# jiahuei/COMIC-Compact-Image-Captioning-with-Attention

Hardware: AMD Instinct MI355X
Metric: images/sec (decoder-mode XE training, COMIC-256, InceptionV3 frozen) (higher is better)
Workload: dtype bf16

## Files before the change

### comic-compact-image-captioning-with-attention_amd/_lib.py

```python
import ctypes as C
import os

_HERE = os.path.dirname(os.path.abspath(__file__))
LIB_PATH = os.environ.get('COMIC_HIP_LIB') or os.path.join(_HERE, 'lib', 'libcomic_hip.so')

c_void_p, c_int, c_int32, c_int64, c_float, c_double, c_char_p, c_uint64 = (
    C.c_void_p, C.c_int, C.c_int32, C.c_int64, C.c_float, C.c_double, C.c_char_p, C.c_uint64)


class CnnOp(C.Structure):
    _fields_ = [(n, c_int32) for n in (
        'kind', 'src', 'dst', 'src_coff', 'dst_coff', 'H', 'W', 'Cin', 'Cout', 'KH', 'KW', 'SH', 'SW',
        'PT', 'PL', 'Ho', 'Wo', 'weight', 'relu', 'out_f32', 'src_f32', 'lane', 'tile', 'group', 'flags', 'min_lds')]


class ImageDesc(C.Structure):
    _fields_ = [('offset', C.c_int64), ('in_h', c_int32), ('in_w', c_int32), ('flip', c_int32), ('oy', c_int32),
                ('ox', c_int32), ('sy', C.c_float), ('sx', C.c_float)]


class ImageAug(C.Structure):
    _fields_ = [('mode', c_int32), ('cy', c_int32), ('cx', c_int32), ('ch', c_int32), ('cw', c_int32), ('sy', C.c_float),
                ('sx', C.c_float), ('ops', C.c_uint8 * 4), ('brightness', C.c_float), ('saturation', C.c_float),
                ('hue', C.c_float), ('contrast', C.c_float)]
# ... 40 lines not shown
            ('COMIC_BWD_OWN_ROWS', '1', DEC_BWD_OWN_ROWS))


def decoder_flags_from_env():
    f = 0
    for name, val, bit in _DEC_ENV:
        if os.environ.get(name, '')[:1] == val:
            f |= bit
    return f


CONV_TILES = 61
WS_TILE = 54
IMG_TILE = 55
CHAIN_TILE = 62
OP_RAW, OP_POOLED_SRC, OP_X3 = 1, 2, 4
OP_CHAIN_LINK = 8
OP_CHAIN_KEEP = 16
IM2COL_CONV_TILES = 12


def is_im2col_tile(tile):
    return tile <= IM2COL_CONV_TILES or 26 <= tile <= 47
PARAM_NAMES = ('W_init', 'K', 'b', 'W_m', 'W_v', 'W_q', 'v', 'ln_g', 'ln_b', 'tau', 'W_a', 'W_o', 'b_o', 'emb', 'cell_ln', 'K_c', 'b_c', 'status')


class DecoderParams(C.Structure):
    _fields_ = [(n, c_void_p) for n in PARAM_NAMES]


# ... 329 lines not shown
```

### comic-compact-image-captioning-with-attention_amd/csrc/conv.hip

```cpp
#include "conv_run.h"
#include "conv_ws.h"
#include "conv_stem.h"
#include "conv_img.h"
#include <cstdlib>
#include <cstring>
#include <algorithm>
#include <vector>

namespace {

template <typename T, int BM, int BN, int WM, int WN, bool MASK = false>
__global__ __launch_bounds__(256) void conv_igemm_kernel(ConvArgs a) {
  constexpr int EPC = Elem<T>::EPC;
  constexpr int BKE = 4 * EPC;
  constexpr int A_PASSES = (BM + 63) / 64;
  constexpr int B_PASSES = (BN + 63) / 64;
  constexpr int TM = BM / WM / 16;
  constexpr int TN = BN / WN / 16;
  static_assert(WM * WN == 4, "4 waves");

  __shared__ __attribute__((aligned(16))) unsigned char smem[2 * (BM + BN) * kRowBytes];
  unsigned char* Xs = smem;
  unsigned char* Ws = smem + 2 * BM * kRowBytes;

// ... 1564 lines not shown
    if (img_config(a[j]) != cfg || !img_same_shape(a[j], a[0])) {
      comic_set_error("conv: the members of an image-resident launch must have one shape");
      return 3;
    }
    ComicImgMember& m = ia.m[j];
    m.x = (const bf16_t*)a[j].x; m.wf = (const bf16_t*)a[j].w_frag; m.scale = a[j].scale; m.shift = a[j].shift; m.y = a[j].y;
    m.x_cs = a[j].x_cs; m.x_co = a[j].x_co; m.y_cs = a[j].y_cs; m.y_co = a[j].y_co;
    m.KH = a[j].KH; m.KW = a[j].KW; m.PT = a[j].PT; m.PL = a[j].PL; m.relu = a[j].relu; m.out_f32 = a[j].out_f32;
  }
  return comic_img_launch(cfg, ia, st);
}

int validate_grouped_conv(const comic_cnn_op* op, int xc, int yc, const comic_conv_weight* wt, int batch);
template <typename HT>
int launch_img_chains(const comic_cnn_op* op, int n, void* const* buffers, const int32_t* buf_channels,
                      const comic_conv_weight* weights, int batch, hipStream_t st) {
  ComicChainArgs ca;
  memset(&ca, 0, sizeof(ca));
  ca.f16 = std::is_same<HT, f16_t>::value;
  ca.B = batch; ca.H = op[0].H; ca.W = op[0].W; ca.Cin = op[0].Cin;
  const int pxb = ca.Cin * 2;
  ca.PXBp = pxb + ((pxb % 64 == 0) ? 32 : 0);
  COMIC_REQUIRE(comic_img_chain_supported(ca.H, ca.W, ca.Cin), "conv chain: %dx%d maps of %d channels are not supported", ca.H,
                ca.W, ca.Cin);
  int nm = 0;
  for (int j = 0; j < n;) {
    COMIC_REQUIRE(nm < kChainMaxMembers, "conv chain: more than %d chains in one launch", kChainMaxMembers);
    ComicChainMember& m = ca.m[nm];
    int len = 0;
    for (;; ++len) {
      COMIC_REQUIRE(j + len < n && len < kChainMaxConvs, "conv chain: a chain of more than %d convs, or a link flag on the last op",
                    kChainMaxConvs);
      const comic_cnn_op* o = op + j + len;
      const comic_conv_weight* wt = weights + o->weight;
      const bool link = (o->flags & COMIC_OP_CHAIN_LINK) != 0;
      if (int rc = validate_grouped_conv(o, buf_channels[o->src], buf_channels[o->dst], wt, batch)) return rc;
      COMIC_REQUIRE(o->SH == 1 && o->SW == 1 && o->Ho == o->H && o->Wo == o->W && o->H == ca.H && o->W == ca.W &&
                        o->Cin == ca.Cin && o->KH * o->KW >= 2 && o->KH * o->KW <= 32 && !(o->flags & (COMIC_OP_RAW | COMIC_OP_X3)),
                    "conv chain: every conv must be a stride-1 SAME conv with BatchNorm over the chain's %dx%dx%d input", ca.H, ca.W,
                    ca.Cin);
// ... 11 lines not shown
        COMIC_REQUIRE(buffers[o->dst] && buf_channels[o->dst] % 4 == 0, "conv chain: a kept intermediate map needs its buffer");
        c.keep = buffers[o->dst]; c.keep_cs = buf_channels[o->dst]; c.keep_co = o->dst_coff;
      }
      if (len == 0) {
        COMIC_REQUIRE(buf_channels[o->src] % 8 == 0 && o->src_coff % 8 == 0 && buffers[o->src], "conv chain: bad source slice");
        m.x = (const bf16_t*)buffers[o->src]; m.x_cs = buf_channels[o->src]; m.x_co = o->src_coff;
      }
      if (!link) {
        COMIC_REQUIRE(buffers[o->dst], "conv chain: null destination");
        m.y = buffers[o->dst]; m.y_cs = buf_channels[o->dst]; m.y_co = o->dst_coff; m.out_f32 = o->out_f32;
        ++len;
        break;
      }
    }
    m.n_convs = len;
    j += len;
    ++nm;
  }
  if (nm == 2 && ca.m[1].n_convs > ca.m[0].n_convs) std::swap(ca.m[0], ca.m[1]);
  ca.n_members = nm;
  return comic_img_chain_launch(ca, st);
}

constexpr int kNumConvTiles = 12;
constexpr int kWideTile0 = 26, kNumWideTiles = 22;
constexpr int kWalkTile0 = 56, kNumWalkTiles = 6;
inline int walk_split(int t) { return t >= kWalkTile0 + 3 ? 2 : 1; }
inline bool is_walk_tile(int t) { return t >= kWalkTile0 && t < kWalkTile0 + kNumWalkTiles; }
inline bool is_im2col_tile(int t) { return t <= kNumConvTiles || (t >= kWideTile0 && t < kWideTile0 + kNumWideTiles) || is_walk_tile(t); }
template <typename HT>
int launch_dma_tile(int tile, const ConvArgs& a, hipStream_t st) {
  switch (tile) {
    case 26: return launch_dma<HT, 128, 128, 2, 2, 2>(a, st);
// ... 174 lines not shown
    t0 += q.Cout / 16;
  }
  a.n_tiles = t0;
  if (int rc = comic_ws_launch(a, st)) return rc;
  COMIC_LAUNCH_CHECK("conv_ws");
  return 0;
}
bool ws_group_selected(const comic_cnn_op* ops, int n, int batch) {
  if (!ws_group_eligible(ops, n)) return false;
  if (ops[0].flags & COMIC_OP_POOLED_SRC) return true;
  if (ops[0].tile == COMIC_WS_TILE) return true;
  return ops[0].tile == 0 && (long)batch * ops[0].Ho * ops[0].Wo >= 64L * 256;
}

int group_tile(const comic_cnn_op* ops, int n, int batch) {
  if (ops[0].tile == COMIC_IMG_TILE || ops[0].tile == COMIC_CHAIN_TILE) return ops[0].tile;
  if (ops[0].tile > 0 && ops[0].tile < COMIC_WS_TILE) return ops[0].tile;
  if (is_walk_tile(ops[0].tile)) return ops[0].tile;
  bool all128 = true;
  for (int i = 0; i < n; ++i) all128 = all128 && ops[i].Cout % 128 == 0;
  auto blocks = [&](int t) {
    long b = 0;
    for (int i = 0; i < n; ++i)
      b += (long)cdiv(batch * ops[i].Ho * ops[i].Wo, kTileBM[t]) * cdiv(ops[i].Cout, kTileBN[t]);
    return b;
  };
  if (all128 && blocks(1) >= 512) return 1;
  if (blocks(2) >= 512) return 2;
  if (blocks(3) >= 384) return 3;
  return 4;
}
// ... 317 lines not shown
    if (ops[i].group <= 0) {
      ++i;
      continue;
    }
    if (ws_group_selected(ops + i, n, batch)) {
      memset(out, 0, sizeof(ConvArgs) * n);
      out += n;
      i += n;
      continue;
    }
    COMIC_REQUIRE(ops[i].tile != COMIC_WS_TILE, "conv: group is not eligible for the weight-stationary 1x1 kernel");
    const int tile = group_tile(ops + i, n, batch);
    for (int j = 0; j < n; ++j)
      COMIC_REQUIRE(tile == COMIC_CHAIN_TILE || !(ops[i + j].flags & COMIC_OP_CHAIN_LINK),
                    "conv: COMIC_OP_CHAIN_LINK ops depend on each other -- their group runs on COMIC_CHAIN_TILE only (got tile %d)", tile);
    if (tile == COMIC_IMG_TILE || tile == COMIC_CHAIN_TILE) {
      memset(out, 0, sizeof(ConvArgs) * n);
      out += n;
      i += n;
      continue;
    }
    int blk = 0;
    for (int j = 0; j < n; ++j) {
      const comic_cnn_op* op = ops + i + j;
      const comic_conv_weight* wt = weights + op->weight;
      if (int rc = validate_grouped_conv(op, buf_channels[op->src], buf_channels[op->dst], wt, batch)) return rc;
      COMIC_REQUIRE(buffers[op->src] && buffers[op->dst], "grouped conv: null buffer");
      ConvArgs& a = out[j];
      fill_args(a, op, buffers[op->src], buf_channels[op->src], buffers[op->dst], buf_channels[op->dst], wt, batch);
      COMIC_REQUIRE(a.zero, "conv: zero page symbol not resolvable");
      a.member_kind = op->kind == 7 ? 1 : 0;
// ... 107 lines not shown
    if (gargs && op->group > 0) {
      COMIC_REQUIRE(dtype == Half16<HT>::code && (op->kind == 0 || op->kind == 7) && op->lane == 0,
                    "grouped launch needs a bf16 or f16 plan and conv / pool+bn ops on the caller's stream");
      const int n = group_run(ops, n_ops, i);
      if (ws_group_selected(op, n, batch)) {
        if (int rc = run_ws_group<HT>(op, n, buffers, buf_channels, weights, batch, main_st)) return rc;
        gargs += n;
        i += n - 1;
        continue;
      }
      COMIC_REQUIRE(op->tile != COMIC_WS_TILE, "conv: group is not eligible for the weight-stationary 1x1 kernel");
      const int tile = group_tile(op, n, batch);
      for (int j = 0; j < n; ++j)
        COMIC_REQUIRE(tile == COMIC_CHAIN_TILE || !(op[j].flags & COMIC_OP_CHAIN_LINK),
                      "conv: COMIC_OP_CHAIN_LINK ops depend on each other -- their group runs on COMIC_CHAIN_TILE only (got tile %d)", tile);
      if (tile == COMIC_CHAIN_TILE) {
        if (int rc = launch_img_chains<HT>(op, n, buffers, buf_channels, weights, batch, main_st)) return rc;
        COMIC_LAUNCH_CHECK("image-resident conv chains");
        gargs += n;
        i += n - 1;
        continue;
      }
      if (tile == COMIC_IMG_TILE) {
        COMIC_REQUIRE(n <= kImgMaxMembers, "grouped launch: too many members for the image-resident kernel");
        ConvArgs ma[kImgMaxMembers];
        bool done[kImgMaxMembers] = {false, false, false, false};
        for (int j = 0; j < n; ++j) {
          COMIC_REQUIRE(op[j].kind == 0, "grouped launch: the image-resident kernel takes convolutions only");
          if (int rc = validate_grouped_conv(op + j, buf_channels[op[j].src], buf_channels[op[j].dst], weights + op[j].weight, batch)) return rc;
          fill_args(ma[j], op + j, buffers[op[j].src], buf_channels[op[j].src], buffers[op[j].dst], buf_channels[op[j].dst],
// ... 186 lines not shown
```

### comic-compact-image-captioning-with-attention_amd/csrc/conv_img.h

```cpp
#pragma once
#include "conv_common.h"

constexpr int kImgMaxMembers = 4;

struct ComicImgMember {
  const bf16_t* x;
  const bf16_t* wf;
  const float* scale;
  const float* shift;
  void* y;
  int x_cs, x_co, y_cs, y_co;
  int KH, KW, PT, PL, relu, out_f32;
};
struct ComicImgArgs {
  ComicImgMember m[kImgMaxMembers];
  int n_members;
  int B, H, W, Cin, Cout;
  int G, groups;
  int PXBp;
  int KS32;
  int f16;
};

int comic_img_config(int H, int W, int Cin, int Cout, int KH, int KW, int SH, int SW, int Ho, int Wo);
// ... 2 lines not shown

constexpr int kChainMaxConvs = 4, kChainMaxMembers = 2;
struct ComicChainConv {
  const bf16_t* wf;
  const float* scale;
  const float* shift;
  int KH, KW, PT, PL, KS32, Cout, relu, keep_cs;
  void* keep;
  int keep_co, pad_;
};
struct ComicChainMember {
  const bf16_t* x;
  void* y;
  int x_cs, x_co, y_cs, y_co, out_f32, n_convs;
  ComicChainConv c[kChainMaxConvs];
};
struct ComicChainArgs {
  ComicChainMember m[kChainMaxMembers];
  int n_members;
  int B, H, W, Cin, PXBp;
  int f16;
};
int comic_img_chain_supported(int H, int W, int Cin);
int comic_img_chain_launch(const ComicChainArgs& a, hipStream_t st);
```

### comic-compact-image-captioning-with-attention_amd/csrc/conv_img.hip

```cpp
#include <algorithm>

#include "conv_img.h"

namespace {

typedef __attribute__((ext_vector_type(4))) unsigned img_u32x4;

__device__ __forceinline__ __amdgpu_buffer_rsrc_t img_rsrc(const void* p, uint32_t bytes) {
  return __builtin_amdgcn_make_buffer_rsrc((void*)p, 0, (int)bytes, 0x00020000);
}

constexpr int img_zero_bytes(int cs) { return (256 + cs * 64 + 1023) / 1024 * 1024; }

template <int TM>
__device__ __forceinline__ void img_pixel_state(int lane, int wm, int P, int H, int W, int PXBp, int KH, int KW, int PT, int PL,
                                                int img0, uint32_t (&pixaddr)[TM], uint32_t (&mask)[TM], int (&mrow)[TM]) {
  const int fr = lane & 15, fg = lane >> 4;
  const int HW = H * W;
  const float rHW = 1.0f / (float)HW, rW = 1.0f / (float)W;
#pragma unroll
  for (int j = 0; j < TM; ++j) {
    const int p = (wm * TM + j) * 16 + fr;
    const bool pv = p < P;
    const int pp = pv ? p : 0;
// ... 118 lines not shown

  const int fg = lane >> 4;
  uint32_t pixaddr[TM], mask[TM];
  int mrow[TM];
  img_pixel_state<TM>(lane, wm, P, a.H, a.W, PXBp, m.KH, m.KW, m.PT, m.PL, img0, pixaddr, mask, mrow);
  f32x4_t acc[TN][TM];
  img_kloop<HT, TM, TN, CS, PD, true>(smem, zoff, pixaddr, mask, m.wf, a.Cout, a.KS32, m.KH, m.KW, m.PT, m.PL, a.W, PXBp, wn, lane, acc);

  ConvArgs ca;
  ca.scale = m.scale; ca.shift = m.shift; ca.y = m.y; ca.y_cs = m.y_cs; ca.y_co = m.y_co; ca.Cout = a.Cout;
  ca.relu = m.relu; ca.out_f32 = m.out_f32; ca.accum = 0; ca.x3 = 0; ca.x3_src = 0;
  ca.mask_y = nullptr;
  conv_store_tiles<HT, TN, TM>(ca, acc, wn * TN * 16, fg * 4, mrow);
}

template <typename HT, int TM, int TNI, int CS, int PD = 2>
__global__ __launch_bounds__(256, 2) void conv_img_chain_kernel(const ComicChainArgs a) {
  constexpr int NT = 256, WN = 4;
  constexpr int CPP = CS * 4;
  constexpr int PMAX = TM * 16;
  extern __shared__ __attribute__((aligned(16))) unsigned char smem[];
  const int tid = threadIdx.x, lane = tid & 63;
  const int wn = __builtin_amdgcn_readfirstlane(tid >> 6);
  const int mi = (int)blockIdx.x >= a.B ? 1 : 0;
  const int img0 = (int)blockIdx.x - mi * a.B;
  const ComicChainMember& m = a.m[mi];
  const int HW = a.H * a.W;
  const int P = HW;
  const int PXBp = a.PXBp;
  const uint32_t zoff = (PMAX * PXBp + 255) & ~255;

  {
    constexpr int U = (PMAX * CPP + NT - 1) / NT;
    const bf16_t* __restrict__ xg = m.x + (size_t)img0 * HW * m.x_cs + m.x_co;
    const int x_cs = m.x_cs;
    const int total = P * CPP;
    uint4 v[U];
    int dst[U];
#pragma unroll
    for (int u = 0; u < U; ++u) {
      const int idx = u * NT + tid;
      const bool ok = idx < total;
      const int p = ok ? idx / CPP : 0;
      const int c = ok ? idx - p * CPP : 0;
      dst[u] = ok ? p * PXBp + c * 16 : -1;
      v[u] = *(const uint4*)(xg + (size_t)p * x_cs + c * 8);
    }
#pragma unroll
    for (int u = 0; u < U; ++u)
      if (dst[u] >= 0) *(uint4*)(smem + dst[u]) = v[u];
    for (int z = tid; z < img_zero_bytes(CS) / 16; z += NT) *(uint4*)(smem + zoff + z * 16) = make_uint4(0u, 0u, 0u, 0u);
  }
  __syncthreads();

  const int fr = lane & 15, fg = lane >> 4;
  uint32_t pixaddr[TM], mask[TM];
  int mrow[TM];
  const int nc = m.n_convs;
  for (int ci = 0; ci + 1 < nc; ++ci) {
    const ComicChainConv& c = m.c[ci];
    img_pixel_state<TM>(lane, 0, P, a.H, a.W, PXBp, c.KH, c.KW, c.PT, c.PL, img0, pixaddr, mask, mrow);
    f32x4_t acc[TNI][TM];
    img_kloop<HT, TM, TNI, CS, PD, false>(smem, zoff, pixaddr, mask, c.wf, a.Cin, c.KS32, c.KH, c.KW, c.PT, c.PL, a.W, PXBp, wn, lane, acc);
    float4 sc[TNI], sh[TNI];
    bool nv[TNI];
#pragma unroll
    for (int i = 0; i < TNI; ++i) {
      nv[i] = (wn * TNI + i) * 16 < a.Cin;
      const int n0 = nv[i] ? (wn * TNI + i) * 16 + fg * 4 : 0;
      sc[i] = *(const float4*)(c.scale + n0);
      sh[i] = *(const float4*)(c.shift + n0);
    }
    const float lo = c.relu ? 0.f : -INFINITY;
    __syncthreads();
#pragma unroll
    for (int j = 0; j < TM; ++j) {
      unsigned char* prow = smem + (j * 16 + fr) * PXBp + (wn * TNI * 16 + fg * 4) * 2;
#pragma unroll
      for (int i = 0; i < TNI; ++i) {
        float v0 = fmaf(acc[i][j][0], sc[i].x, sh[i].x);
        float v1 = fmaf(acc[i][j][1], sc[i].y, sh[i].y);
        float v2 = fmaf(acc[i][j][2], sc[i].z, sh[i].z);
        float v3 = fmaf(acc[i][j][3], sc[i].w, sh[i].w);
        asm("v_max_f32 %0, %1, %2" : "=v"(v0) : "v"(v0), "s"(lo));
        asm("v_max_f32 %0, %1, %2" : "=v"(v1) : "v"(v1), "s"(lo));
        asm("v_max_f32 %0, %1, %2" : "=v"(v2) : "v"(v2), "s"(lo));
        asm("v_max_f32 %0, %1, %2" : "=v"(v3) : "v"(v3), "s"(lo));
        const uint2 pk = make_uint2(Half16<HT>::pack(v0, v1), Half16<HT>::pack(v2, v3));
        if (nv[i]) *(uint2*)(prow + i * 32) = pk;
        if (c.keep && nv[i])
          *(uint2*)((unsigned char*)c.keep + ((size_t)(img0 * HW + j * 16 + fr) * c.keep_cs + c.keep_co + (wn * TNI + i) * 16 + fg * 4) * 2) = pk;
      }
    }
    __syncthreads();
  }
  {
    const ComicChainConv& c = m.c[nc - 1];
    img_pixel_state<TM>(lane, 0, P, a.H, a.W, PXBp, c.KH, c.KW, c.PT, c.PL, img0, pixaddr, mask, mrow);
    f32x4_t acc[3][TM];
    img_kloop<HT, TM, 3, CS, PD, false>(smem, zoff, pixaddr, mask, c.wf, c.Cout, c.KS32, c.KH, c.KW, c.PT, c.PL, a.W, PXBp, wn, lane, acc);
    ConvArgs ca;
    ca.scale = c.scale; ca.shift = c.shift; ca.y = m.y; ca.y_cs = m.y_cs; ca.y_co = m.y_co; ca.Cout = c.Cout;
    ca.relu = c.relu; ca.out_f32 = m.out_f32; ca.accum = 0; ca.x3 = 0; ca.x3_src = 0;
    ca.mask_y = nullptr;
    conv_store_tiles<HT, 3, TM>(ca, acc, wn * 3 * 16, fg * 4, mrow);
  }
}

__global__ void pack_frag_kernel(const bf16_t* __restrict__ src, bf16_t* __restrict__ dst, const long* __restrict__ table,
// ... 39 lines not shown
  if (!attr_set) {
    if (hipFuncSetAttribute((const void*)conv_img_kernel<HT, TM, TN, WM, WN, CS, PD>, hipFuncAttributeMaxDynamicSharedMemorySize,
                            160 * 1024) != hipSuccess) {
      comic_set_error("conv_img: cannot reserve %d bytes of LDS", lds);
      return 1;
    }
    attr_set = true;
  }
  hipLaunchKernelGGL((conv_img_kernel<HT, TM, TN, WM, WN, CS, PD>), dim3(a.groups * a.n_members), dim3(64 * WM * WN), lds, st, a);
  return 0;
}

template <typename HT, int TNI, int CS>
int launch_chain(const ComicChainArgs& a, hipStream_t st) {
  constexpr int TM = 9;
  const int lds = ((TM * 16 * a.PXBp + 255) & ~255) + img_zero_bytes(CS);
  static PerDeviceOnce attr_once__;
  bool& attr_set = attr_once__.slot();
  if (!attr_set) {
    if (hipFuncSetAttribute((const void*)conv_img_chain_kernel<HT, TM, TNI, CS>, hipFuncAttributeMaxDynamicSharedMemorySize,
                            160 * 1024) != hipSuccess) {
      comic_set_error("conv_img_chain: cannot reserve %d bytes of LDS", lds);
      return 1;
    }
    attr_set = true;
  }
  hipLaunchKernelGGL((conv_img_chain_kernel<HT, TM, TNI, CS>), dim3(a.B * a.n_members), dim3(256), lds, st, a);
  return 0;
}

}
// ... 71 lines not shown
```

### comic-compact-image-captioning-with-attention_amd/nets.py

```python
from __future__ import annotations

import ctypes as C
import json
import math
import os

import numpy as np

from . import _lib as L
from . import streams

BN_EPS = 1e-3

_STEM = [('c', 'Conv2d_1a_3x3', 32, (3, 3), 2, 'VALID'), ('c', 'Conv2d_2a_3x3', 32, (3, 3), 1, 'VALID'),
         ('c', 'Conv2d_2b_3x3', 64, (3, 3), 1, 'SAME'), ('max', 'MaxPool_3a_3x3'),
         ('c', 'Conv2d_3b_1x1', 80, (1, 1), 1, 'VALID'), ('c', 'Conv2d_4a_3x3', 192, (3, 3), 1, 'VALID'),
         ('max', 'MaxPool_5a_3x3')]


def _c(scope, cout, k, stride=1, pad='SAME'):
    return ('c', scope, cout, k if isinstance(k, tuple) else (k, k), stride, pad)


def _mixed5(pool_c, b1):
# ... 67 lines not shown
            and 2 * (32 + 64) * 4 + 2 * 4 * 132 * 96 + 16 * Wi * 3 * 4 <= 160 * 1024)


def _out(size, k, s, pad):
    if pad == 'SAME':
        o = -(-size // s)
        tot = max((o - 1) * s + k - size, 0)
        return o, tot // 2
    return (size - k) // s + 1, 0


class CnnPlan:

    def __init__(self, name='inception_v3', image_size=(224, 224), final_endpoint='Mixed_7c', branch_streams=False,
                 group_branches=True, layers=None, pool_after_projection=False, ride_pools=False, side_pools=None,
                 fuse_pools=False, x3=False, fuse_stem_1a=True, fuse_chains=None):
        if name not in ('inception_v3', 'inception_v1', 'chain'):
            raise NotImplementedError('only inception_v3 / inception_v1 are on the MI355X hot path (got %r)' % name)
        self.name = name
        self.ops = []
        self.buffers = []
        self.weights = []
        self.wphys = []
        self.fm_src = None
        self.end_points = {}
        self.macs = 0
        self._lane = 0
        self._branch = None
        self.branch_streams = branch_streams
        self.group_branches = group_branches and not branch_streams
        self._depth = 0
        self._next_group = 1
        self.pool_after_projection = pool_after_projection
        self.ride_pools = ride_pools
        self.side_pools = bool(side_pools)
        self.fuse_pools = bool(fuse_pools)
        self.fuse_stem_1a = bool(fuse_stem_1a)
        bf16_grouped = not x3 and self.group_branches and name == 'inception_v3' and not self.ride_pools
        self.fuse_chains = bf16_grouped if fuse_chains is None else bool(fuse_chains)
        self.keep_chain_maps = not self.pool_after_projection
        self.small_batch_plan = None
        if fuse_chains is None and self.fuse_chains:
            self.small_batch_plan = CnnPlan(name, image_size, final_endpoint, branch_streams, group_branches, layers,
                                            pool_after_projection, ride_pools, side_pools, fuse_pools, x3, fuse_stem_1a,
                                            fuse_chains=False)
        if self.fuse_chains and (x3 or not self.group_branches):
            raise ValueError('fuse_chains needs a grouped bf16 plan')
        if self.fuse_pools and not (pool_after_projection and name == 'inception_v3'):
            raise ValueError('fuse_pools needs an inception_v3 plan with pool_after_projection=True')
        self._pooled_src = None
        self._logical = {}
        self.block_ranges = []
        if name == 'chain':
            self._build_chain(image_size, layers)
        elif name == 'inception_v1':
# ... 91 lines not shown
                             KH=k, KW=k, SH=stride, SW=stride, PT=pt, PL=pl, Ho=Ho, Wo=Wo, weight=-1, relu=0,
                             out_f32=0, lane=self._lane, depth=self._depth, branch=self._branch))
        return dst, (Ho, Wo, Cc)

    def _schedule_by_depth(self, first_op):
        block = self.ops[first_op:]
        del self.ops[first_op:]
        forked = False
        chains = self._find_chains(block) if self.fuse_chains else []
        chained = [o for ch in chains for o in ch]
        for ch in chains:
            rest = sorted((o for o in block if o.get('branch') == ch[0].get('branch') and o['depth'] > ch[-1]['depth']),
                          key=lambda o: o['depth'])
            for k, o in enumerate(rest):
                o['depth'] = ch[0]['depth'] + k
        block = [o for o in block if not any(o is c for c in chained)]
        for di, d in enumerate(sorted({o['depth'] for o in block})):
            if di == 1 and chains:
                self._emit_chains(chains)
                chains = []
            level = [o for o in block if o['depth'] == d]
            riders = [o for o in level if o['kind'] == 7] if self.ride_pools else []
            for o in level:
                if o['kind'] != 0 and o not in riders:
                    if o['kind'] == 7 and self.side_pools:
                        o['lane'] = 1
                        self.ops.append(self._sync_op(5))
                        forked = True
                    self.ops.append(o)
            convs = sorted((o for o in level if o['kind'] == 0), key=lambda o: -(o['KH'] * o['KW'] * o['Cin']))
            if not convs:
                self.ops += riders
                continue
            members = convs + riders
            if len(members) >= 2:
                for o in members:
                    o['group'] = self._next_group
                self._next_group += 1
            self.ops += members
        if chains:
            self._emit_chains(chains)
        if forked:
            self.ops.append(self._sync_op(6))

    CHAIN_CHANNELS = (128, 160, 192)
    CHAIN_MIN_BATCH = 96

    def _find_chains(self, block):
        def seven(o, cin):
            return (o['kind'] == 0 and o['H'] * o['W'] == 144 and (o['Ho'], o['Wo']) == (o['H'], o['W']) and
                    o['SH'] == o['SW'] == 1 and o['KH'] * o['KW'] == 7 and o['Cin'] == cin and not o.get('flags', 0))
        out = []
        for b in sorted({o.get('branch') for o in block if o.get('branch') is not None}):
            ops = sorted((o for o in block if o.get('branch') == b), key=lambda o: o['depth'])
            if len(ops) < 3 or ops[0]['kind'] != 0:
                continue
# ... 2 lines not shown
            for o in ops[1:]:
                if not (cin in self.CHAIN_CHANNELS and seven(o, cin) and len(run) < 4):
                    break
                if run and not (run[-1]['Cout'] == cin and not run[-1]['out_f32'] and run[-1]['dst'] == o['src']
                                and run[-1]['dst_coff'] == 0 and sum(1 for q in block if q['src'] == run[-1]['dst']) == 1):
                    break
                run.append(o)
            while run and run[-1]['Cout'] != 192:
                run.pop()
            if len(run) >= 2:
                out.append(run)
        if len(out) > 2 or len({ch[0]['Cin'] for ch in out}) > 1:
            return []
        return out

    def _emit_chains(self, chains):
        for ch in chains:
            for o in ch[:-1]:
                o['flags'] = o.get('flags', 0) | L.OP_CHAIN_LINK | (L.OP_CHAIN_KEEP if self.keep_chain_maps else 0)
            for o in ch:
                o['group'] = self._next_group
                o['tile'] = L.CHAIN_TILE
                self.ops.append(o)
        self._next_group += 1

    @staticmethod
    def _sync_op(kind):
        z = dict.fromkeys(('src', 'dst', 'src_coff', 'dst_coff', 'H', 'W', 'Cin', 'Cout', 'KH', 'KW', 'SH', 'SW', 'PT',
                           'PL', 'Ho', 'Wo', 'relu', 'out_f32'), 0)
        z.update(kind=kind, weight=-1, lane=0)
        return z
# ... 377 lines not shown
        self._train = None
        torch.cuda.synchronize()
        self._wt = wt
        self.bufs = []
        for (H, W, Cc, f32) in plan.buffers:
            self.bufs.append(torch.empty((batch, H, W, Cc), dtype=torch.float32 if f32 else tdt, device=device))
        self._bufptr = (C.c_void_p * len(self.bufs))(*[b.data_ptr() for b in self.bufs])
        self._bufch = (C.c_int32 * len(self.bufs))(*[b[2] for b in plan.buffers])
        ops = (L.CnnOp * len(plan.ops))()
        for i, o in enumerate(plan.ops):
            for k, v in o.items():
                if k not in ('depth', 'branch', 'block_in'):
                    setattr(ops[i], k, v)
            if not self.half:
                ops[i].group = 0
                if o.get('tile') == L.CHAIN_TILE:
                    ops[i].tile = 0
                    ops[i].flags &= ~(L.OP_CHAIN_LINK | L.OP_CHAIN_KEEP)
        self._ops = ops
        self._group_args = None
        self._build_group_args()
        self._graph = None
        self._calls = 0
        self._alt = {}
        self._last_bufptr = None
        self.backward_lanes = True
        self.backward_branch_lanes = True
        self._polite_lds_kb = 0
        self._fm_f32 = None

    @property
# ... 401 lines not shown
            src = self.bufs[self.plan.fm_src]
            if self._fm_f32 is None:
                self._fm_f32 = self.torch.empty(src.shape, dtype=self.torch.float32, device=self.device)
            self._fm_f32.copy_(src)
            fm = self._fm_f32
        else:
            fm = self.bufs[self.plan.fm]
        return pooled.reshape(B, -1), fm.reshape(B, fm.shape[1] * fm.shape[2], fm.shape[3])

    def _tune_key(self):
        p = self.plan
        H, W = p.buffers[p.input][:2]
        return '%s:%dx%d:B%d:%s%s:%dops:polite%d' % (p.name, H, W, self.batch, 'par' if p.pool_after_projection else 'plain',
                                                    ('+fp' if getattr(p, 'fuse_pools', False) else '') +
                                                    ('+ch' if getattr(p, 'fuse_chains', False) else '') +
                                                    ('+x3' if getattr(p, 'x3', False) else ''),
                                                  len(p.ops), self.polite_lds_kb) + (':f16' if self.dtype == 'f16' else '')

    def autotune(self, reps=5, verbose=False, cache=None):
        if not self.half:
            return {}
        torch = self.torch
        st = L.stream_ptr()
        if cache and os.path.isfile(cache):
            tiles = json.load(open(cache)).get(self._tune_key())
            if tiles is not None and len(tiles) == len(self.plan.ops):
                for i, t in enumerate(tiles):
                    self._ops[i].tile = int(t)
                if self._group_args is not None:
                    self._build_group_args()
# ... 9 lines not shown
        ev0, ev1 = torch.cuda.Event(enable_timing=True), torch.cuda.Event(enable_timing=True)
        n_ops = len(self.plan.ops)
        grouped = self._group_args is not None
        rec_bytes = 0
        if grouped:
            n_rec = sum(1 for j in range(n_ops) if self._ops[j].group > 0)
            rec_bytes = self.lib.comic_cnn_group_args_bytes(self._ops, n_ops) // n_rec
        rec = 0
        i = 0
        while i < n_ops:
            o = self.plan.ops[i]
            if o['kind'] != 0:
                i += 1
                continue
            op = self._ops[i]
            if o.get('flags', 0) & L.OP_POOLED_SRC or o.get('tile') == L.CHAIN_TILE:
                n = 1
                while i + n < n_ops and op.group > 0 and self._ops[i + n].group == op.group:
                    n += 1
                rec += n if (grouped and op.group > 0) else 0
                i += n
                continue
            n = 1
            if grouped and op.group > 0:
                while i + n < n_ops and self._ops[i + n].group == op.group:
                    n += 1
                first = C.byref(self._ops, i * C.sizeof(L.CnnOp))
                rec_off = rec * rec_bytes

                def run():
                    L.check(self.lib.comic_cnn_forward_grouped(first, n, self._bufptr, self._bufch, self._wt,
# ... 83 lines not shown
```

### include/comic_hip.h

```cpp
#ifndef COMIC_HIP_H_
#define COMIC_HIP_H_

#include <stddef.h>
#include <stdint.h>

#ifdef __cplusplus
extern "C" {
#endif

#define COMIC_F32 0
#define COMIC_BF16 1
#define COMIC_F16 2
#define COMIC_ABI_VERSION 1
#define COMIC_CONV_TILES 61
#define COMIC_WS_TILE 54
#define COMIC_IMG_TILE 55
#define COMIC_CHAIN_TILE 62

const char* comic_last_error(void);
int comic_abi_version(void);
int comic_device_count(void);


int comic_pack_conv_weights(const float* w_hwio, void* w_packed, int kh, int kw, int cin, int cout,
                            int dtype, void* stream);

int comic_fold_bn(const float* beta, const float* mean, const float* var, float eps, float* scale,
                  float* shift, int c, void* stream);

typedef struct comic_cnn_op {
  int32_t kind;
  int32_t src, dst;
// ... 597 lines not shown
```

Baseline: 40330.

## Fuse 1x1 head convs into image-resident conv chain kernels

```diff
diff --git a/comic-compact-image-captioning-with-attention_amd/_lib.py b/comic-compact-image-captioning-with-attention_amd/_lib.py
--- a/comic-compact-image-captioning-with-attention_amd/_lib.py
+++ b/comic-compact-image-captioning-with-attention_amd/_lib.py
@@ -78,6 +78,7 @@
 WS_TILE = 54
 IMG_TILE = 55
 CHAIN_TILE = 62
+CHAIN_HEAD_TILE = 63
 OP_RAW, OP_POOLED_SRC, OP_X3 = 1, 2, 4
 OP_CHAIN_LINK = 8
 OP_CHAIN_KEEP = 16
diff --git a/comic-compact-image-captioning-with-attention_amd/csrc/conv.hip b/comic-compact-image-captioning-with-attention_amd/csrc/conv.hip
--- a/comic-compact-image-captioning-with-attention_amd/csrc/conv.hip
+++ b/comic-compact-image-captioning-with-attention_amd/csrc/conv.hip
@@ -1602,7 +1602,8 @@
 int validate_grouped_conv(const comic_cnn_op* op, int xc, int yc, const comic_conv_weight* wt, int batch);
 template <typename HT>
 int launch_img_chains(const comic_cnn_op* op, int n, void* const* buffers, const int32_t* buf_channels,
-                      const comic_conv_weight* weights, int batch, hipStream_t st) {
+                      const comic_conv_weight* weights, int batch, hipStream_t st, const comic_cnn_op* heads = nullptr,
+                      int n_heads = 0) {
   ComicChainArgs ca;
   memset(&ca, 0, sizeof(ca));
   ca.f16 = std::is_same<HT, f16_t>::value;
@@ -1611,7 +1612,7 @@
   ca.PXBp = pxb + ((pxb % 64 == 0) ? 32 : 0);
   COMIC_REQUIRE(comic_img_chain_supported(ca.H, ca.W, ca.Cin), "conv chain: %dx%d maps of %d channels are not supported", ca.H,
                 ca.W, ca.Cin);
-  int nm = 0;
+  int nm = 0, heads_used = 0;
   for (int j = 0; j < n;) {
     COMIC_REQUIRE(nm < kChainMaxMembers, "conv chain: more than %d chains in one launch", kChainMaxMembers);
     ComicChainMember& m = ca.m[nm];
@@ -1653,9 +1654,40 @@
       }
     }
     m.n_convs = len;
+    for (int h = 0; h < n_heads; ++h) {
+      const comic_cnn_op* o = heads + h;
+      if (o->dst != op[j].src) continue;
+      const comic_conv_weight* wt = weights + o->weight;
+      COMIC_REQUIRE(!m.head.wf, "conv chain: two heads write the input of one chain");
+      if (int rc = validate_grouped_conv(o, buf_channels[o->src], buf_channels[o->dst], wt, batch)) return rc;
+      COMIC_REQUIRE(o->kind == 0 && o->KH == 1 && o->KW == 1 && o->SH == 1 && o->SW == 1 && o->PT == 0 && o->PL == 0 &&
+                        o->H == ca.H && o->W == ca.W && o->Ho == ca.H && o->Wo == ca.W && o->Cout == ca.Cin &&
+                        o->Cin % kChainHeadKT == 0 && !(o->flags & ~COMIC_OP_CHAIN_KEEP) && !o->out_f32 && o->dst_coff == 0 &&
+                        buf_channels[o->dst] == ca.Cin,
+                    "conv chain: a head must be a stride-1 1x1 conv with BatchNorm from a multiple of %d channels to the chain's %dx%dx%d map",
+                    kChainHeadKT, ca.H, ca.W, ca.Cin);
+      COMIC_REQUIRE(wt->w_frag, "conv chain: no fragment-order weights");
+      COMIC_REQUIRE(buffers[o->src] && buf_channels[o->src] % 8 == 0 && o->src_coff % 8 == 0 &&
+                        o->src_coff + o->Cin <= buf_channels[o->src],
+                    "conv chain: bad source slice of a head");
+      ComicChainConv& c = m.head;
+      c.wf = (const bf16_t*)wt->w_frag; c.scale = wt->scale; c.shift = wt->shift;
+      c.KH = 1; c.KW = 1; c.PT = 0; c.PL = 0; c.Cout = o->Cout; c.relu = o->relu;
+      c.KS32 = ((o->Cin + 63) / 64 * 64) / 32;
+      c.keep = nullptr;
+      if (o->flags & COMIC_OP_CHAIN_KEEP) {
+        COMIC_REQUIRE(buffers[o->dst] && buf_channels[o->dst] % 4 == 0, "conv chain: a kept intermediate map needs its buffer");
+        c.keep = buffers[o->dst]; c.keep_cs = buf_channels[o->dst]; c.keep_co = o->dst_coff;
+      }
+      m.head_cin = o->Cin;
+      m.x = (const bf16_t*)buffers[o->src]; m.x_cs = buf_channels[o->src]; m.x_co = o->src_coff;
+      ca.heads = 1;
+      ++heads_used;
+    }
     j += len;
     ++nm;
   }
+  COMIC_REQUIRE(heads_used == n_heads, "conv chain: a head feeds no chain of the next group");
   if (nm == 2 && ca.m[1].n_convs > ca.m[0].n_convs) std::swap(ca.m[0], ca.m[1]);
   ca.n_members = nm;
   return comic_img_chain_launch(ca, st);
@@ -1860,7 +1892,7 @@
 }
 
 int group_tile(const comic_cnn_op* ops, int n, int batch) {
-  if (ops[0].tile == COMIC_IMG_TILE || ops[0].tile == COMIC_CHAIN_TILE) return ops[0].tile;
+  if (ops[0].tile == COMIC_IMG_TILE || ops[0].tile == COMIC_CHAIN_TILE || ops[0].tile == COMIC_CHAIN_HEAD_TILE) return ops[0].tile;
   if (ops[0].tile > 0 && ops[0].tile < COMIC_WS_TILE) return ops[0].tile;
   if (is_walk_tile(ops[0].tile)) return ops[0].tile;
   bool all128 = true;
@@ -2208,7 +2240,11 @@
     for (int j = 0; j < n; ++j)
       COMIC_REQUIRE(tile == COMIC_CHAIN_TILE || !(ops[i + j].flags & COMIC_OP_CHAIN_LINK),
                     "conv: COMIC_OP_CHAIN_LINK ops depend on each other -- their group runs on COMIC_CHAIN_TILE only (got tile %d)", tile);
-    if (tile == COMIC_IMG_TILE || tile == COMIC_CHAIN_TILE) {
+    if (tile == COMIC_CHAIN_HEAD_TILE)
+      COMIC_REQUIRE(i + n < n_ops && ops[i + n].group > 0 &&
+                        group_tile(ops + i + n, group_run(ops, n_ops, i + n), batch) == COMIC_CHAIN_TILE,
+                    "conv: a COMIC_CHAIN_HEAD_TILE group must stand in front of the COMIC_CHAIN_TILE group it feeds");
+    if (tile == COMIC_IMG_TILE || tile == COMIC_CHAIN_TILE || tile == COMIC_CHAIN_HEAD_TILE) {
       memset(out, 0, sizeof(ConvArgs) * n);
       out += n;
       i += n;
@@ -2346,6 +2382,16 @@
       for (int j = 0; j < n; ++j)
         COMIC_REQUIRE(tile == COMIC_CHAIN_TILE || !(op[j].flags & COMIC_OP_CHAIN_LINK),
                       "conv: COMIC_OP_CHAIN_LINK ops depend on each other -- their group runs on COMIC_CHAIN_TILE only (got tile %d)", tile);
+      if (tile == COMIC_CHAIN_HEAD_TILE) {
+        COMIC_REQUIRE(i + n < n_ops && op[n].group > 0 && group_tile(op + n, group_run(ops, n_ops, i + n), batch) == COMIC_CHAIN_TILE,
+                      "conv: a COMIC_CHAIN_HEAD_TILE group must stand in front of the COMIC_CHAIN_TILE group it feeds");
+        const int nc = group_run(ops, n_ops, i + n);
+        if (int rc = launch_img_chains<HT>(op + n, nc, buffers, buf_channels, weights, batch, main_st, op, n)) return rc;
+        COMIC_LAUNCH_CHECK("image-resident conv chains with heads");
+        gargs += n + nc;
+        i += n + nc - 1;
+        continue;
+      }
       if (tile == COMIC_CHAIN_TILE) {
         if (int rc = launch_img_chains<HT>(op, n, buffers, buf_channels, weights, batch, main_st)) return rc;
         COMIC_LAUNCH_CHECK("image-resident conv chains");
diff --git a/comic-compact-image-captioning-with-attention_amd/csrc/conv_img.h b/comic-compact-image-captioning-with-attention_amd/csrc/conv_img.h
--- a/comic-compact-image-captioning-with-attention_amd/csrc/conv_img.h
+++ b/comic-compact-image-captioning-with-attention_amd/csrc/conv_img.h
@@ -40,12 +40,16 @@
   void* y;
   int x_cs, x_co, y_cs, y_co, out_f32, n_convs;
   ComicChainConv c[kChainMaxConvs];
+  ComicChainConv head;
+  int head_cin, pad_;
 };
 struct ComicChainArgs {
   ComicChainMember m[kChainMaxMembers];
   int n_members;
   int B, H, W, Cin, PXBp;
   int f16;
+  int heads;
 };
+constexpr int kChainHeadKT = 64;
 int comic_img_chain_supported(int H, int W, int Cin);
 int comic_img_chain_launch(const ComicChainArgs& a, hipStream_t st);
diff --git a/comic-compact-image-captioning-with-attention_amd/csrc/conv_img.hip b/comic-compact-image-captioning-with-attention_amd/csrc/conv_img.hip
--- a/comic-compact-image-captioning-with-attention_amd/csrc/conv_img.hip
+++ b/comic-compact-image-captioning-with-attention_amd/csrc/conv_img.hip
@@ -156,6 +156,142 @@
   conv_store_tiles<HT, TN, TM>(ca, acc, wn * TN * 16, fg * 4, mrow);
 }
 
+constexpr int kHeadPXB = kChainHeadKT * 2 + 32;
+constexpr int kHeadStage = 144 * kHeadPXB;
+constexpr int kHeadRing = 2 * kHeadStage;
+__host__ __device__ constexpr uint32_t chain_zoff(int pmax, int PXBp, int heads) {
+  const uint32_t map = (uint32_t)(pmax * PXBp + 255) & ~255u;
+  return heads && map < (uint32_t)kHeadRing ? (uint32_t)kHeadRing : map;
+}
+
+template <typename HT, int TM, int TN, int PD>
+__device__ __forceinline__ void img_head_kloop(unsigned char* smem, const bf16_t* __restrict__ xg, int x_cs, int head_cin,
+                                               const bf16_t* wf, int Cout, int KS32, int wn, int tid, int lane,
+                                               f32x4_t (&acc)[TN][TM]) {
+  constexpr int NT = 256;
+  constexpr int CPT = kChainHeadKT / 8;
+  constexpr int U = (TM * 16 * CPT + NT - 1) / NT;
+  constexpr int KSTEPS = kChainHeadKT / 32;
+  static_assert(TM * 16 == 144, "the head's stages hold one 12x12 image");
+#pragma unroll
+  for (int i = 0; i < TN; ++i)
+#pragma unroll
+    for (int j = 0; j < TM; ++j) acc[i][j] = (f32x4_t){0.f, 0.f, 0.f, 0.f};
+  const int nkt = head_cin / kChainHeadKT;
+  const __amdgpu_buffer_rsrc_t xr = img_rsrc(xg, (uint32_t)(TM * 16 - 1) * (uint32_t)x_cs * 2u + (uint32_t)head_cin * 2u);
+  int voff[U], dst[U];
+#pragma unroll
+  for (int u = 0; u < U; ++u) {
+    const int idx = u * NT + tid;
+    const bool ok = idx < TM * 16 * CPT;
+    const int p = idx / CPT, c = idx % CPT;
+    voff[u] = ok ? (p * x_cs + c * 8) * 2 : 0x7ffffff0;
+    dst[u] = ok ? p * kHeadPXB + c * 16 : -1;
+  }
+  img_u32x4 va[U], vb[U];
+  auto request = [&](img_u32x4 (&v)[U], int kt) {
+#pragma unroll
+    for (int u = 0; u < U; ++u) v[u] = __builtin_amdgcn_raw_buffer_load_b128(xr, voff[u], kt * (kChainHeadKT * 2), 0);
+  };
+  auto deposit = [&](const img_u32x4 (&v)[U], int kt) {
+    unsigned char* stg = smem + (kt & 1) * kHeadStage;
+#pragma unroll
+    for (int u = 0; u < U; ++u)
+      if (dst[u] >= 0) *(img_u32x4*)(stg + dst[u]) = v[u];
+  };
+  request(va, 0);
+  if (nkt > 1) request(vb, 1);
+
+  const __amdgpu_buffer_rsrc_t wr = img_rsrc(wf, (uint32_t)(Cout / 16) * (uint32_t)KS32 * 1024u);
+  const int wv = lane * 16;
+  const int tile_stride = KS32 * 1024;
+  const int wbase = wn * TN * tile_stride;
+  const int nsteps = nkt * KSTEPS;
+  img_u32x4 wq[PD + 1][TN];
+#pragma unroll
+  for (int d = 0; d < PD; ++d)
+#pragma unroll
+    for (int i = 0; i < TN; ++i)
+      wq[d][i] = __builtin_amdgcn_raw_buffer_load_b128(wr, wv, wbase + min(d, nsteps - 1) * 1024 + i * tile_stride, 0);
+
+  deposit(va, 0);
+  __syncthreads();
+
+  const int fr = lane & 15, fg = lane >> 4;
+  uint4 xf[TM];
+  int s = 0;
+  auto tile = [&](int kt, img_u32x4 (&vfree)[U], const img_u32x4 (&vnext)[U]) {
+    if (kt + 2 < nkt) request(vfree, kt + 2);
+    const unsigned char* st = smem + (kt & 1) * kHeadStage + fr * kHeadPXB + fg * 16;
+#pragma unroll
+    for (int cs = 0; cs < KSTEPS; ++cs) {
+      const int so = wbase + min(s + PD, nsteps - 1) * 1024;
+      ++s;
+#pragma unroll
+      for (int i = 0; i < TN; ++i)
+        wq[PD][i] = __builtin_amdgcn_raw_buffer_load_b128(wr, wv, so + i * tile_stride, 0);
+#pragma unroll
+      for (int j = 0; j < TM; ++j) xf[j] = *(const uint4*)(st + j * 16 * kHeadPXB + cs * 64);
+      __builtin_amdgcn_sched_barrier(0);
+#pragma unroll
+      for (int i = 0; i < TN; ++i)
+#pragma unroll
+        for (int j = 0; j < TM; ++j)
+          acc[i][j] = Half16<HT>::mfma(__builtin_bit_cast(bf16x8_t, wq[0][i]),
+                                                              __builtin_bit_cast(bf16x8_t, xf[j]), acc[i][j]);
+#pragma unroll
+      for (int d = 0; d < PD; ++d)
+#pragma unroll
+        for (int i = 0; i < TN; ++i) wq[d][i] = wq[d + 1][i];
+    }
+    if (kt + 1 < nkt) {
+      deposit(vnext, kt + 1);
+      __syncthreads();
+    }
+  };
+  for (int kt = 0; kt < nkt; kt += 2) {
+    tile(kt, va, vb);
+    if (kt + 1 < nkt) tile(kt + 1, vb, va);
+  }
+}
+
+template <typename HT, int TM, int TNI>
+__device__ __forceinline__ void chain_store_map(unsigned char* smem, const ComicChainConv& c, int Cmap, int PXBp, int wn,
+                                                int lane, int row0, const f32x4_t (&acc)[TNI][TM]) {
+  const int fr = lane & 15, fg = lane >> 4;
+  float4 sc[TNI], sh[TNI];
+  bool nv[TNI];
+#pragma unroll
+  for (int i = 0; i < TNI; ++i) {
+    nv[i] = (wn * TNI + i) * 16 < Cmap;
+    const int n0 = nv[i] ? (wn * TNI + i) * 16 + fg * 4 : 0;
+    sc[i] = *(const float4*)(c.scale + n0);
+    sh[i] = *(const float4*)(c.shift + n0);
+  }
+  const float lo = c.relu ? 0.f : -INFINITY;
+  __syncthreads();
+#pragma unroll
+  for (int j = 0; j < TM; ++j) {
+    unsigned char* prow = smem + (j * 16 + fr) * PXBp + (wn * TNI * 16 + fg * 4) * 2;
+#pragma unroll
+    for (int i = 0; i < TNI; ++i) {
+      float v0 = fmaf(acc[i][j][0], sc[i].x, sh[i].x);
+      float v1 = fmaf(acc[i][j][1], sc[i].y, sh[i].y);
+      float v2 = fmaf(acc[i][j][2], sc[i].z, sh[i].z);
+      float v3 = fmaf(acc[i][j][3], sc[i].w, sh[i].w);
+      asm("v_max_f32 %0, %1, %2" : "=v"(v0) : "v"(v0), "s"(lo));
+      asm("v_max_f32 %0, %1, %2" : "=v"(v1) : "v"(v1), "s"(lo));
+      asm("v_max_f32 %0, %1, %2" : "=v"(v2) : "v"(v2), "s"(lo));
+      asm("v_max_f32 %0, %1, %2" : "=v"(v3) : "v"(v3), "s"(lo));
+      const uint2 pk = make_uint2(Half16<HT>::pack(v0, v1), Half16<HT>::pack(v2, v3));
+      if (nv[i]) *(uint2*)(prow + i * 32) = pk;
+      if (c.keep && nv[i])
+        *(uint2*)((unsigned char*)c.keep + ((size_t)(row0 + j * 16 + fr) * c.keep_cs + c.keep_co + (wn * TNI + i) * 16 + fg * 4) * 2) = pk;
+    }
+  }
+  __syncthreads();
+}
+
 template <typename HT, int TM, int TNI, int CS, int PD = 2>
 __global__ __launch_bounds__(256, 2) void conv_img_chain_kernel(const ComicChainArgs a) {
   constexpr int NT = 256, WN = 4;
@@ -170,9 +306,15 @@
   const int HW = a.H * a.W;
   const int P = HW;
   const int PXBp = a.PXBp;
-  const uint32_t zoff = (PMAX * PXBp + 255) & ~255;
-
-  {
+  const uint32_t zoff = chain_zoff(PMAX, PXBp, a.heads);
+
+  if (m.head.wf) {
+    for (int z = tid; z < img_zero_bytes(CS) / 16; z += NT) *(uint4*)(smem + zoff + z * 16) = make_uint4(0u, 0u, 0u, 0u);
+    f32x4_t acc[TNI][TM];
+    img_head_kloop<HT, TM, TNI, PD>(smem, m.x + (size_t)img0 * HW * m.x_cs + m.x_co, m.x_cs, m.head_cin, m.head.wf, a.Cin,
+                                    m.head.KS32, wn, tid, lane, acc);
+    chain_store_map<HT, TM, TNI>(smem, m.head, a.Cin, PXBp, wn, lane, img0 * HW, acc);
+  } else {
     constexpr int U = (PMAX * CPP + NT - 1) / NT;
     const bf16_t* __restrict__ xg = m.x + (size_t)img0 * HW * m.x_cs + m.x_co;
     const int x_cs = m.x_cs;
@@ -192,10 +334,10 @@
     for (int u = 0; u < U; ++u)
       if (dst[u] >= 0) *(uint4*)(smem + dst[u]) = v[u];
     for (int z = tid; z < img_zero_bytes(CS) / 16; z += NT) *(uint4*)(smem + zoff + z * 16) = make_uint4(0u, 0u, 0u, 0u);
-  }
-  __syncthreads();
-
-  const int fr = lane & 15, fg = lane >> 4;
+    __syncthreads();
+  }
+
+  const int fg = lane >> 4;
   uint32_t pixaddr[TM], mask[TM];
   int mrow[TM];
   const int nc = m.n_convs;
@@ -204,37 +346,7 @@
     img_pixel_state<TM>(lane, 0, P, a.H, a.W, PXBp, c.KH, c.KW, c.PT, c.PL, img0, pixaddr, mask, mrow);
     f32x4_t acc[TNI][TM];
     img_kloop<HT, TM, TNI, CS, PD, false>(smem, zoff, pixaddr, mask, c.wf, a.Cin, c.KS32, c.KH, c.KW, c.PT, c.PL, a.W, PXBp, wn, lane, acc);
-    float4 sc[TNI], sh[TNI];
-    bool nv[TNI];
-#pragma unroll
-    for (int i = 0; i < TNI; ++i) {
-      nv[i] = (wn * TNI + i) * 16 < a.Cin;
-      const int n0 = nv[i] ? (wn * TNI + i) * 16 + fg * 4 : 0;
-      sc[i] = *(const float4*)(c.scale + n0);
-      sh[i] = *(const float4*)(c.shift + n0);
-    }
-    const float lo = c.relu ? 0.f : -INFINITY;
-    __syncthreads();
-#pragma unroll
-    for (int j = 0; j < TM; ++j) {
-      unsigned char* prow = smem + (j * 16 + fr) * PXBp + (wn * TNI * 16 + fg * 4) * 2;
-#pragma unroll
-      for (int i = 0; i < TNI; ++i) {
-        float v0 = fmaf(acc[i][j][0], sc[i].x, sh[i].x);
-        float v1 = fmaf(acc[i][j][1], sc[i].y, sh[i].y);
-        float v2 = fmaf(acc[i][j][2], sc[i].z, sh[i].z);
-        float v3 = fmaf(acc[i][j][3], sc[i].w, sh[i].w);
-        asm("v_max_f32 %0, %1, %2" : "=v"(v0) : "v"(v0), "s"(lo));
-        asm("v_max_f32 %0, %1, %2" : "=v"(v1) : "v"(v1), "s"(lo));
-        asm("v_max_f32 %0, %1, %2" : "=v"(v2) : "v"(v2), "s"(lo));
-        asm("v_max_f32 %0, %1, %2" : "=v"(v3) : "v"(v3), "s"(lo));
-        const uint2 pk = make_uint2(Half16<HT>::pack(v0, v1), Half16<HT>::pack(v2, v3));
-        if (nv[i]) *(uint2*)(prow + i * 32) = pk;
-        if (c.keep && nv[i])
-          *(uint2*)((unsigned char*)c.keep + ((size_t)(img0 * HW + j * 16 + fr) * c.keep_cs + c.keep_co + (wn * TNI + i) * 16 + fg * 4) * 2) = pk;
-      }
-    }
-    __syncthreads();
+    chain_store_map<HT, TM, TNI>(smem, c, a.Cin, PXBp, wn, lane, img0 * HW, acc);
   }
   {
     const ComicChainConv& c = m.c[nc - 1];
@@ -304,7 +416,7 @@
 template <typename HT, int TNI, int CS>
 int launch_chain(const ComicChainArgs& a, hipStream_t st) {
   constexpr int TM = 9;
-  const int lds = ((TM * 16 * a.PXBp + 255) & ~255) + img_zero_bytes(CS);
+  const int lds = (int)chain_zoff(TM * 16, a.PXBp, a.heads) + img_zero_bytes(CS);
   static PerDeviceOnce attr_once__;
   bool& attr_set = attr_once__.slot();
   if (!attr_set) {
diff --git a/comic-compact-image-captioning-with-attention_amd/nets.py b/comic-compact-image-captioning-with-attention_amd/nets.py
--- a/comic-compact-image-captioning-with-attention_amd/nets.py
+++ b/comic-compact-image-captioning-with-attention_amd/nets.py
@@ -105,7 +105,7 @@
 
     def __init__(self, name='inception_v3', image_size=(224, 224), final_endpoint='Mixed_7c', branch_streams=False,
                  group_branches=True, layers=None, pool_after_projection=False, ride_pools=False, side_pools=None,
-                 fuse_pools=False, x3=False, fuse_stem_1a=True, fuse_chains=None):
+                 fuse_pools=False, x3=False, fuse_stem_1a=True, fuse_chains=None, chain_heads=None):
         if name not in ('inception_v3', 'inception_v1', 'chain'):
             raise NotImplementedError('only inception_v3 / inception_v1 are on the MI355X hot path (got %r)' % name)
         self.name = name
@@ -130,6 +130,9 @@
         bf16_grouped = not x3 and self.group_branches and name == 'inception_v3' and not self.ride_pools
         self.fuse_chains = bf16_grouped if fuse_chains is None else bool(fuse_chains)
         self.keep_chain_maps = not self.pool_after_projection
+        self.chain_heads = self.fuse_chains if chain_heads is None else bool(chain_heads)
+        if self.chain_heads and not self.fuse_chains:
+            raise ValueError('chain_heads needs fuse_chains')
         self.small_batch_plan = None
         if fuse_chains is None and self.fuse_chains:
             self.small_batch_plan = CnnPlan(name, image_size, final_endpoint, branch_streams, group_branches, layers,
@@ -251,10 +254,12 @@
                           key=lambda o: o['depth'])
             for k, o in enumerate(rest):
                 o['depth'] = ch[0]['depth'] + k
+        heads = [self._chain_head(block, ch) for ch in chains] if self.chain_heads else []
+        chained += [h for h in heads if h is not None]
         block = [o for o in block if not any(o is c for c in chained)]
         for di, d in enumerate(sorted({o['depth'] for o in block})):
             if di == 1 and chains:
-                self._emit_chains(chains)
+                self._emit_chains(chains, heads)
                 chains = []
             level = [o for o in block if o['depth'] == d]
             riders = [o for o in level if o['kind'] == 7] if self.ride_pools else []
@@ -276,7 +281,7 @@
                 self._next_group += 1
             self.ops += members
         if chains:
-            self._emit_chains(chains)
+            self._emit_chains(chains, heads)
         if forked:
             self.ops.append(self._sync_op(6))
 
@@ -309,7 +314,28 @@
             return []
         return out
 
-    def _emit_chains(self, chains):
+    @staticmethod
+    def _chain_head(block, ch):
+        first = ch[0]
+        prod = [o for o in block if o['dst'] == first['src'] and o is not first]
+        if len(prod) != 1:
+            return None
+        h = prod[0]
+        ok = (h['kind'] == 0 and (h['KH'], h['KW'], h['SH'], h['SW']) == (1, 1, 1, 1) and (h['Ho'], h['Wo']) == (h['H'], h['W'])
+              and (h['H'], h['W']) == (first['H'], first['W']) and h['Cin'] % 64 == 0 and h['Cout'] == first['Cin']
+              and not h['out_f32'] and h['dst_coff'] == 0 and not h.get('flags', 0) and h.get('branch') == first.get('branch')
+              and sum(1 for q in block if q['src'] == h['dst']) == 1)
+        return h if ok else None
+
+    def _emit_chains(self, chains, heads=()):
+        heads = [h for h in heads if h is not None]
+        for h in heads:
+            h['flags'] = h.get('flags', 0) | (L.OP_CHAIN_KEEP if self.keep_chain_maps else 0)
+            h['group'] = self._next_group
+            h['tile'] = L.CHAIN_HEAD_TILE
+            self.ops.append(h)
+        if heads:
+            self._next_group += 1
         for ch in chains:
             for o in ch[:-1]:
                 o['flags'] = o.get('flags', 0) | L.OP_CHAIN_LINK | (L.OP_CHAIN_KEEP if self.keep_chain_maps else 0)
@@ -717,7 +743,7 @@
                     setattr(ops[i], k, v)
             if not self.half:
                 ops[i].group = 0
-                if o.get('tile') == L.CHAIN_TILE:
+                if o.get('tile') in (L.CHAIN_TILE, L.CHAIN_HEAD_TILE):
                     ops[i].tile = 0
                     ops[i].flags &= ~(L.OP_CHAIN_LINK | L.OP_CHAIN_KEEP)
         self._ops = ops
@@ -1149,6 +1175,7 @@
         return '%s:%dx%d:B%d:%s%s:%dops:polite%d' % (p.name, H, W, self.batch, 'par' if p.pool_after_projection else 'plain',
                                                     ('+fp' if getattr(p, 'fuse_pools', False) else '') +
                                                     ('+ch' if getattr(p, 'fuse_chains', False) else '') +
+                                                    ('+hd' if getattr(p, 'chain_heads', False) else '') +
                                                     ('+x3' if getattr(p, 'x3', False) else ''),
                                                   len(p.ops), self.polite_lds_kb) + (':f16' if self.dtype == 'f16' else '')
 
@@ -1188,7 +1215,7 @@
                 i += 1
                 continue
             op = self._ops[i]
-            if o.get('flags', 0) & L.OP_POOLED_SRC or o.get('tile') == L.CHAIN_TILE:
+            if o.get('flags', 0) & L.OP_POOLED_SRC or o.get('tile') in (L.CHAIN_TILE, L.CHAIN_HEAD_TILE):
                 n = 1
                 while i + n < n_ops and op.group > 0 and self._ops[i + n].group == op.group:
                     n += 1
diff --git a/include/comic_hip.h b/include/comic_hip.h
--- a/include/comic_hip.h
+++ b/include/comic_hip.h
@@ -16,6 +16,7 @@
 #define COMIC_WS_TILE 54
 #define COMIC_IMG_TILE 55
 #define COMIC_CHAIN_TILE 62
+#define COMIC_CHAIN_HEAD_TILE 63
 
 const char* comic_last_error(void);
 int comic_abi_version(void);
```

Result: no change. 40660, median of 6 (+0.8%).
